# shz9/viprs

Hardware: AMD Instinct MI355X
Metric: SNP-updates/sec/E-step (1M SNPs, ~1700 LD blocks) (higher is better)
Workload: dtype f32

## Files before the change

### viprs_amd/csrc/estep_panel.h

```cpp
#pragma once
#include <type_traits>

#include "device_math.h"
#include "kernels_common.h"
#include "panel_loads.h"
#include "panel_models.h"

#ifndef PANEL_MIN_WAVES
#define PANEL_MIN_WAVES 2
#endif

namespace viprs {

#ifdef VIPRS_SWEEP_TRACE
__device__ unsigned long long g_sweep_trace[1 << 15][4];
__device__ unsigned int g_sweep_trace_n;
#endif

#ifdef VIPRS_PANEL_PROFILE
#define PPROF(slot, cond) do { if (TEAM && item == 0 && member < 2 && lane == 0 && p < 64 && (cond)) s_pprof[p][slot] = (unsigned)wall_clock64(); } while (0)
#else
#define PPROF(slot, cond) do { } while (0)
#endif

template <typename U> __host__ __device__ constexpr int panel_cols() { return sizeof(U) == 4 ? 4 : 8; }
template <typename U> __host__ __device__ constexpr int panel_team_cols() {
#ifdef PANEL_TEAM_CPL_F32
    return sizeof(U) == 4 ? PANEL_TEAM_CPL_F32 : 4;
#else
    return sizeof(U) == 4 ? 2 : 4;
#endif
}

constexpr int kFormSym = 1, kFormMirror = 2;

template <typename U, typename MODEL, int FORM, int NW, bool TEAM, int CPL>
__device__ __forceinline__ void panel_role(const EStepArgs<float>& A0, const int qcap, float* __restrict__ smem, const int wg) {
    constexpr bool MIR = FORM == kFormMirror;
    constexpr bool SUMS = FORM != kFormSym;
    const PanelLds lds(qcap, MODEL::kLaneParallel && !is_wide_mixture<MODEL>::value, MIR);
    float* lq = smem + lds.q();
    float* la = smem + lds.a();
    float* lT = smem + lds.diag_tiles();
    float* lTo = smem + lds.offdiag_tile();
    float* lmx = smem + lds.mix();
    float* led = smem + lds.ed();
    float* ls = smem + lds.s();
#ifdef PANEL_TEAM_STRIP_DEPTH
    constexpr int kDepth = TEAM ? PANEL_TEAM_STRIP_DEPTH : kStripRowsInFlight;
#else
    constexpr int kDepth = TEAM ? (kPanel / RawRow<U, CPL>::kWords < kPanel ? kPanel / RawRow<U, CPL>::kWords : kPanel) : kStripRowsInFlight;
#endif
    __shared__ int s_blk;
    __shared__ int s_tdone;
    __shared__ int s_ddone;

    const int tid = threadIdx.x;
    const int wave = __builtin_amdgcn_readfirstlane(tid >> 6);
    const int lane = tid & 63;
    const U* __restrict__ ldd = static_cast<const U*>(A0.ld_dense);
    ExpTab tab;
    tab.init();
    unsigned long long my_skipped = 0;
    const float dq = A0.dq;
    const int n_models = max(1, A0.n_active);

    constexpr int kSW = kPanel * CPL;
    const int TS = TEAM ? A0.team_size : 1;
    const int team = TEAM ? wg / TS : 0;
    const int member = TEAM ? wg % TS : 0;
    int team_iter = 0;

    for (;;) {
        int item;
        if (TEAM) {
            item = team + team_iter * A0.n_teams;
            ++team_iter;
        } else {
            if (tid == 0) {
                int it = atomicAdd(A0.counter, 1);
                if (A0.bottom_mod > 0 && it < A0.n_blocks * n_models) {
                    const bool bottom = (wg % A0.bottom_mod) == A0.bottom_mod - 1;
                    it = bottom ? A0.n_blocks * n_models - 1 - atomicAdd(A0.counter + 2, 1) : atomicAdd(A0.counter + 1, 1);
                }
                s_blk = it;
            }
            __syncthreads();
            item = s_blk;
            __syncthreads();
        }
        if (item >= A0.n_blocks * n_models) break;
        const int blk = item / n_models, model_slot = item - blk * n_models;
        if constexpr (IsGridColumn<MODEL>::value) {
            if (A0.group_cols) {
                const int on = A0.group_cols[(int64_t)A0.blk_group[blk] * A0.width + A0.active[model_slot]];
                if (__builtin_amdgcn_readfirstlane(on) == 0) continue;
            }
        }
        const EStepArgs<float> A = select_model(A0, model_slot);

        const BlockDesc bd = A.blocks[blk];
        const int64_t s0 = bd.start;
        const int b = bd.size;
#ifdef VIPRS_SWEEP_TRACE
        const unsigned long long trace_t0 = wall_clock64();
#endif
        unsigned long long* __restrict__ gran =
            TEAM ? A.granules + ((int64_t)model_slot * A.granule_rows + bd.gr_off) * kPanel : nullptr;
        const int stride = bd.stride;
        const U* __restrict__ base = ldd + bd.ld_off;
        const int np = (b + kPanel - 1) / kPanel;
        const int bpad = np * kPanel;
        const int nstrips_all = (bpad + kSW - 1) / kSW;
        const int n_own = TEAM ? (nstrips_all - member + TS - 1) / TS : nstrips_all;
        auto own = [&](int c) { return !TEAM || ((c / kSW) % TS) == member; };
        auto loc = [&](int c) { return TEAM ? ((c / kSW) / TS) * kSW + (c % kSW) : c; };
        auto glob = [&](int li) { return TEAM ? ((li / kSW) * TS + member) * kSW + (li % kSW) : li; };

        for (int li = tid; li < (TEAM ? n_own * kSW : bpad) + kStrip; li += NW * 64) {
            const int c = glob(li);
            const bool in = (!TEAM || li < n_own * kSW) && c < b;
            lq[li] = in ? A.q[s0 + c] : 0.0f;
            if (SUMS) ls[li] = 0.0f;
        }
        if (tid == 0) { s_tdone = 0; s_ddone = 0; }
        for (int i = tid; i < kPanel * kPanel / 4; i += NW * 64) {
            const int row = i >> 4, tcol = (i & 15) * 4;
            *reinterpret_cast<float4*>(lT + row * kPanel + tcol) = load4<U>(base + (int64_t)min(row, b - 1) * stride + tcol);
        }
        __syncthreads();

        float a_prev = 0.0f;

        typename MODEL::In nxt_in{};
        if (wave == 0) {
            const bool live0 = lane < b;
            nxt_in = MODEL::load(A, s0 + (live0 ? lane : 0), live0);
        }

#ifdef VIPRS_PANEL_PROFILE
        __shared__ unsigned s_pprof[64][8];
#endif
        if (wave == 0) {
#ifdef PANEL_CHAIN_PRIO
        __builtin_amdgcn_s_setprio(PANEL_CHAIN_PRIO);
#endif
        for (int p = 0; p < np + 1; ++p) {
            PPROF(0, true);
            {
                if (p < np) {
                    const int r0 = p * kPanel;
                    const int nrows = min(kPanel, b - r0);
                    const int64_t j = s0 + r0 + lane;
                    const bool live = lane < nrows;
                    const typename MODEL::In in = nxt_in;
                    {
                        const int rn = r0 + kPanel + lane;
                        const bool ln = rn < b;
                        nxt_in = MODEL::load(A, s0 + (ln ? rn : 0), ln);
                    }

                    float qc;
                    float q_own = 0.0f;
                    if (own(r0)) qc = lq[loc(r0 + lane)];
                    else qc = (r0 + lane < b) ? A.q[s0 + r0 + lane] : 0.0f;
                    if (TEAM && p >= 2 && (((p * kPanel) / kSW) % TS) != member) {
                        unsigned long long g = 0;
#ifdef PANEL_TIMING_NO_HANDOFF_WAIT
                        if (false)
#endif
                        for (unsigned spins = 0;; ++spins) {
                            g = __hip_atomic_load(gran + (int64_t)p * kPanel + lane, __ATOMIC_RELAXED,
                                                  __HIP_MEMORY_SCOPE_AGENT);
                            if (__all((unsigned)(g >> 32) == A.tag_base + (unsigned)(p + 1))) break;
                            if (spins > (1u << 22)) {
                                if (lane == 0) atomicExch(A.error, 1);
                                break;
                            }
                            if ((spins & 1023u) == 1023u &&
                                __hip_atomic_load(A.error, __ATOMIC_RELAXED, __HIP_MEMORY_SCOPE_AGENT) != 0) break;
                            __builtin_amdgcn_s_sleep(8);
                        }
                        qc = __uint_as_float((unsigned)g);
                    }
                    PPROF(1, true);
                    if (p > 0) {
                        {
                            float trow[kPanel];
#pragma unroll
                            for (int k = 0; k < kPanel; ++k) trow[k] = lTo[k * kPanel + lane];
                            if constexpr (sizeof(U) < 4 || MODEL::kLaneParallel) {
                                const float4* __restrict__ av4 = reinterpret_cast<const float4*>(la + ((p - 1) & 1) * kPanel);
                                float4 av[kPanel / 4];
#pragma unroll
                                for (int i = 0; i < kPanel / 4; ++i) av[i] = av4[i];
#pragma unroll
                                for (int k = 0; k < kPanel; ++k) {
                                    const float4 t = av[k >> 2];
                                    const float ak = (k & 3) == 0 ? t.x : (k & 3) == 1 ? t.y : (k & 3) == 2 ? t.z : t.w;
                                    qc = __builtin_fmaf(trow[k], ak, qc);
                                }
                            } else {
#pragma unroll
                                for (int k = 0; k < kPanel; ++k) qc = __builtin_fmaf(trow[k], rl(a_prev, k), qc);
                            }
                        }
                    }

                    {
                        if (lane == 0) *reinterpret_cast<volatile int*>(&s_tdone) = p + 1;
                    }
                    PPROF(2, true);
                    if constexpr (is_wide_mixture<MODEL>::value) {
                        constexpr int KMAX = MODEL::kMax;
                        const int K = in.K;
                        const int kc = min(lane, K - 1);
                        const bool comp = lane < K;
                        float dvec = 0.0f, avec = 0.0f;
                        const int64_t jlast = s0 + b - 1;
                        auto cptr = [&](const float* __restrict__ arr, int jj) {
                            return arr + min(s0 + r0 + jj, jlast) * K + kc;
                        };
                        static_assert(kChainPrefetch == 16 && kPanel == 64, "window indexing");
                        float rmm[kChainPrefetch], rsv[kChainPrefetch], rul[kChainPrefetch];
                        float rvec = in.beta - qc;
                        const float* __restrict__ DtW = lT + (p & 1) * kPanel * kPanel + lane;
#pragma unroll
                        for (int k = 0; k < kChainPrefetch; ++k) {
                            rmm[k] = *cptr(A.mu_mult, k);
                            rsv[k] = *cptr(A.shvt, k);
                            rul[k] = *cptr(A.u_logs, k);
                        }
#pragma unroll 1
                        for (int g = 0; g < kPanel / kChainPrefetch; ++g) {
#pragma unroll
                        for (int k = 0; k < kChainPrefetch; ++k) {
                            const int jj = kChainPrefetch * g + k;
                            const float drow_jj = DtW[jj * kPanel];
                            const float cmm = rmm[k], csv = rsv[k], cul = rul[k];
                            {
                                rmm[k] = *cptr(A.mu_mult, jj + kChainPrefetch);
                                rsv[k] = *cptr(A.shvt, jj + kChainPrefetch);
                                rul[k] = *cptr(A.u_logs, jj + kChainPrefetch);
                            }
                            const float lnp = rl(in.lnp, jj), eta_old = rl(in.eta_old, jj);
                            const float r = rl(rvec, jj);
                            const float mu = cmm * r;
                            const float t = csv * mu;
                            float u = __builtin_fmaf(t, t, cul);
                            u = (lane == K) ? lnp : u;
                            float mx = dpp_max_shr<1>(u);
                            mx = dpp_max_shr<2>(mx);
                            mx = dpp_max_shr<4>(mx);
                            mx = dpp_max_shr<8>(mx);
                            const float m_lo = rl(mx, 15), m_hi = rl(mx, K);
                            mx = (K >= 16) ? fmaxf(m_lo, m_hi) : m_hi;
                            float e = expf_glibc_nonpos<kLookupPerLane>(u - mx, tab);
                            e = (lane <= K) ? e : 0.0f;
                            static_assert((KMAX + 1) % 8 == 0, "chunks of 8 terms");
                            float ssum = 0.0f;
#pragma unroll
                            for (int c = 0; c < (KMAX + 1) / 8; ++c) {
                                int et[8];
#pragma unroll
                                for (int i = 0; i < 8; ++i) et[i] = __builtin_amdgcn_readlane(__float_as_int(e), 8 * c + i);
                                pin_sgprs(et);
#pragma unroll
                                for (int i = 0; i < 8; ++i) ssum = (c == 0 && i == 0) ? __int_as_float(et[0]) : ssum + __int_as_float(et[i]);
                            }
                            const float gam = comp ? e / ssum : 0.0f;
                            float d = -eta_old;
#pragma unroll
                            for (int c = 0; c < (KMAX + 1) / 8; ++c) {
                                int gt[8];
                                float mb[8];
#pragma unroll
                                for (int i = 0; i < 8; ++i) {
                                    gt[i] = __builtin_amdgcn_readlane(__float_as_int(gam), 8 * c + i);
                                    mb[i] = rl(mu, 8 * c + i);
                                }
                                pin_sgprs(gt);
#pragma unroll
                                for (int i = 0; i < 8; ++i) d = __builtin_fmaf(__int_as_float(gt[i]), mb[i], d);
                            }
                            const bool livej = jj < nrows;
                            const float a = livej ? dq * d : 0.0f;
                            if (comp && livej && member == 0) {
                                const int64_t o = (s0 + r0 + jj) * K + lane;
                                A.var_mu[o] = mu;
                                A.var_gamma[o] = gam;
                            }
                            int l = lane;
                            asm volatile("" : "+v"(l));
                            const bool me = (l == jj);
                            dvec = me ? d : dvec;
                            avec = me ? a : avec;
                            if (MIR) q_own = me ? qc : q_own;
                            qc = __builtin_fmaf(drow_jj, a, qc);
                            rvec = in.beta - qc;
                            if (!MIR) qc = (me && livej) ? qc - d : qc;
                        }
                        }
                        if (member == 0 && live) {
                            A.eta_diff[j] = dvec;
                            if (TEAM) stage_store(A.eta_out + j, in.eta_old + dvec); else A.eta[j] = in.eta_old + dvec;
                        }
                        a_prev = avec;
                        if (SUMS) led[(p & 1) * kPanel + lane] = live ? dvec : 0.0f;
                    } else if constexpr (MODEL::kLaneParallel) {
                        const int K = in.K;
                        float* __restrict__ Lmm = lmx;
                        float* __restrict__ Lsv = lmx + kPanel * kPanelMaxK;
                        float* __restrict__ Lul = lmx + 2 * kPanel * kPanelMaxK;
                        float* __restrict__ Lmu = lmx + 3 * kPanel * kPanelMaxK;
                        float* __restrict__ Lga = lmx + 4 * kPanel * kPanelMaxK;
#pragma unroll
                        for (int k = 0; k < kPanelMaxK; ++k) {
                            if (k < K) {
                                Lmm[lane * K + k] = in.mm[k];
                                Lsv[lane * K + k] = in.sv[k];
                                Lul[lane * K + k] = in.ulog[k];
                            }
                        }
                        __builtin_amdgcn_wave_barrier();
                        const int kc = min(lane, K - 1);
                        float cmm = Lmm[kc], csv = Lsv[kc], cul = Lul[kc];
                        float dvec = 0.0f, avec = 0.0f;
                        auto run_panel = [&](auto rounds_c, auto k4_c) {
                        constexpr int ROUNDS = decltype(rounds_c)::value;
                        constexpr bool K4 = decltype(k4_c)::value;
                        float rvec = in.beta - qc;
                        static_assert(kChainPrefetch == 16 && kPanel == 64, "group indexing");
                        const float* __restrict__ Dt = lT + (p & 1) * kPanel * kPanel + lane;
#pragma unroll 1
                        for (int g = 0; g < kPanel / kChainPrefetch; ++g) {
#pragma unroll
                        for (int k = 0; k < kChainPrefetch; ++k) {
                            const int jj = kChainPrefetch * g + k;
                            const float drow_jj = Dt[jj * kPanel];
                            const int jn = (jj + 1 < kPanel) ? jj + 1 : jj;
                            const float nmm = Lmm[jn * K + kc], nsv = Lsv[jn * K + kc], nul = Lul[jn * K + kc];
                            const float lnp = rl(in.lnp, jj), eta_old = rl(in.eta_old, jj);
                            const float r = rl(rvec, jj);
                            const float mu = cmm * r;
                            const float t = csv * mu;
                            float u = __builtin_fmaf(t, t, cul);
                            u = (lane == K) ? lnp : u;
                            float mub[ROUNDS];
#pragma unroll
                            for (int i = 0; i < ROUNDS; ++i) mub[i] = rl(mu, i);
                            float mx;
                            if constexpr (K4) {
                                int ut[5];
#pragma unroll
                                for (int i = 0; i < 5; ++i) ut[i] = __builtin_amdgcn_readlane(__float_as_int(u), i);
                                pin_sgprs(ut);
                                mx = __int_as_float(ut[0]);
#pragma unroll
                                for (int i = 1; i <= 4; ++i) mx = fmaxf(mx, __int_as_float(ut[i]));
                            } else {
                                mx = dpp_max_shr<1>(u);
                                mx = dpp_max_shr<2>(mx);
                                mx = dpp_max_shr<4>(mx);
                                mx = dpp_max_shr<8>(mx);
                                mx = rl(mx, K);
                            }
                            const float e = softmax_exp<MODEL::kExact, kLookupPerLane>(u - mx, tab);
                            const float e_t = (K4 || lane <= K) ? e : 0.0f;
                            int et[ROUNDS + 1];
#pragma unroll
                            for (int i = 0; i <= ROUNDS; ++i) et[i] = __builtin_amdgcn_readlane(__float_as_int(e_t), i);
                            pin_sgprs(et);
                            float ssum = __int_as_float(et[0]);
#pragma unroll
                            for (int i = 1; i <= ROUNDS; ++i) ssum += __int_as_float(et[i]);
                            const float gam = softmax_div<MODEL::kExact>(e, ssum);
                            const float gam_t = (K4 || lane < K) ? gam : 0.0f;
                            int gt[ROUNDS];
#pragma unroll
                            for (int i = 0; i < ROUNDS; ++i) gt[i] = __builtin_amdgcn_readlane(__float_as_int(gam_t), i);
                            pin_sgprs(gt);
                            float d = -eta_old;
#pragma unroll
                            for (int i = 0; i < ROUNDS; ++i) d = __builtin_fmaf(__int_as_float(gt[i]), mub[i], d);
                            const bool livej = jj < nrows;
                            const float a = livej ? dq * d : 0.0f;
                            if (lane < K) {
                                Lmu[jj * K + lane] = mu;
                                Lga[jj * K + lane] = gam;
                            }
                            int l = lane;
                            asm volatile("" : "+v"(l));
                            const bool me = (l == jj);
                            dvec = me ? d : dvec;
                            avec = me ? a : avec;
                            if (MIR) q_own = me ? qc : q_own;
                            qc = __builtin_fmaf(drow_jj, a, qc);
                            rvec = in.beta - qc;
                            if (!MIR) qc = (me && livej) ? qc - d : qc;
                            cmm = nmm; csv = nsv; cul = nul;
                        }
                        }
                        };
                        if (K == 4) run_panel(std::integral_constant<int, 4>{}, std::true_type{});
                        else if (K < 4) run_panel(std::integral_constant<int, 4>{}, std::false_type{});
                        else run_panel(std::integral_constant<int, kPanelMaxK>{}, std::false_type{});
                        __builtin_amdgcn_wave_barrier();
                        if (member == 0) {
                            const int64_t o = (s0 + r0) * K;
                            for (int i = lane; i < nrows * K; i += 64) {
                                A.var_mu[o + i] = Lmu[i];
                                A.var_gamma[o + i] = Lga[i];
                            }
                            if (live) {
                                A.eta_diff[j] = dvec;
                                if (TEAM) stage_store(A.eta_out + j, in.eta_old + dvec); else A.eta[j] = in.eta_old + dvec;
                            }
                        }
                        a_prev = avec;
                        if (SUMS) led[(p & 1) * kPanel + lane] = live ? dvec : 0.0f;
                    } else {
                        float qcap_v = 0.0f;
                        const float* __restrict__ Dt = lT + (p & 1) * kPanel * kPanel + lane;
                        unsigned long long lane_bit = 1ull;
                        float qf = qc;
    #pragma unroll
                        for (int jj = 0; jj < kPanel; ++jj) {
                            const float dr = Dt[jj * kPanel];
                            const float d = MODEL::template delta<kLookupLane>(in, qf, tab, jj);
                            const float dz = (MODEL::kHasSkip && fabsf(d) < Eps<float>::value) ? 0.0f : d;
                            const float az = dq * dz;
                            const float sa = rl(az, jj);
                            const float sdz = rl(dz, jj);
                            qcap_v = sel_mask(qcap_v, qc, lane_bit);
                            qf = __builtin_fmaf(dr, sa, qc);
                            qc = !MIR ? sel_mask(qf, qf - sdz, lane_bit) : qf;
                            asm volatile("s_lshl_b64 %0, %0, 1" : "+s"(lane_bit) : : "scc");
                        }
                        q_own = qcap_v;

                        PPROF(3, true);
                        bool skipped_lane;
                        float d_lane = 0.0f;
                        a_prev = MODEL::template finish<TEAM>(A, j, in, qcap_v, tab, live, member == 0, skipped_lane, &d_lane);
                        my_skipped += __popcll(__ballot(skipped_lane));
                        if (SUMS) led[(p & 1) * kPanel + lane] = d_lane;
                    }
                    la[(p & 1) * kPanel + lane] = a_prev;
                    if (own(r0)) lq[loc(r0 + lane)] = MIR ? q_own : qc;
                    PPROF(4, true);
                }
            }
            __syncthreads();
        }
        } else {
        for (int p = 0; p < np + 1; ++p) {
            {
                const int uw = wave - 1;
                auto stage_tiles = [&]() {
                if (p + 1 < np) {
                    float* __restrict__ T = lT + ((p + 1) & 1) * kPanel * kPanel;
                    const int trow = lane >> 4, tcol = (lane & 15) * 4;
                    const int row_base = (p + 1) * kPanel;
                    constexpr int kGroups = (kPanel / 4 + NW - 2) / (NW - 1);
                    float4 v[kGroups];
#pragma unroll
                    for (int g = 0; g < kGroups; ++g) {
                        const int row = 4 * min(uw + g * (NW - 1), kPanel / 4 - 1) + trow;
                        v[g] = load4<U>(base + (int64_t)min(row_base + row, b - 1) * stride + (p + 1) * kPanel + tcol);
                    }
                    float4 w[kGroups];
                    {
#pragma unroll
                        for (int g = 0; g < kGroups; ++g) {
                            const int row = 4 * min(uw + g * (NW - 1), kPanel / 4 - 1) + trow;
                            w[g] = load4<U>(base + (int64_t)min(p * kPanel + row, b - 1) * stride + (p + 1) * kPanel + tcol);
                        }
                    }
                    if (MIR && p > 0) {
                        while (*reinterpret_cast<volatile int*>(&s_ddone) < p) __builtin_amdgcn_s_sleep(1);
                    }
#pragma unroll
                    for (int g = 0; g < kGroups; ++g) {
                        const int i = uw + g * (NW - 1);
                        if (i < kPanel / 4) *reinterpret_cast<float4*>(T + (4 * i + trow) * kPanel + tcol) = v[g];
                    }
                    {
                        while (*reinterpret_cast<volatile int*>(&s_tdone) < p + 1) __builtin_amdgcn_s_sleep(1);
#pragma unroll
                        for (int g = 0; g < kGroups; ++g) {
                            const int i = uw + g * (NW - 1);
                            if (i < kPanel / 4) *reinterpret_cast<float4*>(lTo + (4 * i + trow) * kPanel + tcol) = w[g];
                        }
                    }
                }
                };
                const int pp = p - 1;
                const int rr0 = pp * kPanel;
                const int last_row = min(kPanel, b - rr0) - 1;
                const float avec = p > 0 ? la[(pp & 1) * kPanel + lane] : 0.0f;
                const int nstrips = (bpad + kSW - 1) / kSW;
                const bool any_a = __ballot(avec != 0.0f) != 0;
                const float edvec = (MIR && p > 0) ? led[(pp & 1) * kPanel + lane] : 0.0f;
                const bool any_ed = MIR && __ballot(edvec != 0.0f) != 0;
                const int s_pri = ((p + 1) * kPanel) / kSW;
                const int n_mine = (nstrips - member + TS - 1) / TS;
                auto do_strip = [&](int k) {
                    int st = member + k * TS, kl = k;
                    if (TEAM) {
                        const int k_pri = (s_pri % TS == member) ? (s_pri - member) / TS : 0;
                        kl = (k + k_pri) % n_mine;
                        st = member + kl * TS;
                    }
                    const int c = st * kSW + CPL * lane;
                    float* __restrict__ lq_c = lq + (TEAM ? kl * kSW + CPL * lane : c);
                    const int cp = c >> 6;
#if defined(PANEL_TIMING_NO_SECOND_PASS) && PANEL_TIMING_NO_SECOND_PASS + 0 >= 2
                    const bool active = (c < b) && cp > p;
#else
                    const bool active = (c < b) && cp != pp && cp != p;
#endif
                    auto hand_off = [&]() {
                        if (TEAM && st == s_pri && p + 1 < np && p + 1 >= 2) {
                            __builtin_amdgcn_wave_barrier();
                            const float v = lq[loc((p + 1) * kPanel + lane)];
                            const unsigned long long g =
                                ((unsigned long long)(A.tag_base + (unsigned)(p + 2)) << 32) | (unsigned long long)__float_as_uint(v);
                            __hip_atomic_store(gran + (int64_t)(p + 1) * kPanel + lane, g, __ATOMIC_RELAXED,
                                               __HIP_MEMORY_SCOPE_AGENT);
                        }
                    };
                    if constexpr (MIR) {
                        const bool left = cp < pp;
                        float* __restrict__ tgt = left ? ls + (TEAM ? kl * kSW + CPL * lane : c) : lq_c;
                        const bool any_l = __ballot(active && left) != 0, any_r = __ballot(active && !left) != 0;
                        if (any_l && any_r) {
                            const float fvec = left ? 1.0f : dq;
                            if (any_ed && active) {
                                if (last_row == kPanel - 1)
                                    strip_update<U, CPL, true, kDepth, true>(base + (int64_t)rr0 * stride + c, stride, last_row, edvec, tgt, fvec);
                                else
                                    strip_update<U, CPL, false, kDepth, true>(base + (int64_t)rr0 * stride + c, stride, last_row, edvec, tgt, fvec);
                            }
                        } else {
                            float mvec = any_l ? edvec : avec;
                            asm volatile("" : "+v"(mvec));
                            if ((any_l ? any_ed : any_a) && active) {
                                if (last_row == kPanel - 1)
                                    strip_update<U, CPL, true, kDepth>(base + (int64_t)rr0 * stride + c, stride, last_row, mvec, tgt);
                                else
                                    strip_update<U, CPL, false, kDepth>(base + (int64_t)rr0 * stride + c, stride, last_row, mvec, tgt);
                            }
                        }
                        if (k == uw) PPROF(6, wave == 1);
                        hand_off();
                    } else {
                        if (any_a && active) {
                            if (last_row == kPanel - 1)
                                strip_update<U, CPL, true, kDepth>(base + (int64_t)rr0 * stride + c, stride, last_row, avec, lq_c);
                            else
                                strip_update<U, CPL, false, kDepth>(base + (int64_t)rr0 * stride + c, stride, last_row, avec, lq_c);
                        }
                        if (k == uw) PPROF(6, wave == 1);
                        hand_off();
                    }
                };
                if (MIR && p > 0 && uw == NW - 2) {
#ifdef PANEL_TIMING_NO_SECOND_PASS
                    if (false) {
#else
                    if (any_ed && own(rr0)) {
#endif
                        float* __restrict__ sp = ls + loc(rr0 + lane);
                        *sp = diag_lower_update(lT + (pp & 1) * kPanel * kPanel, edvec, *sp, lane);
                    }
                    if (lane == 0) *reinterpret_cast<volatile int*>(&s_ddone) = p;
                }
                stage_tiles();
                PPROF(5, wave == 1);
                if (p > 0) {
                    for (int k = uw; k < n_mine; k += NW - 1) do_strip(k);
                }
            }
            PPROF(7, wave == 1);
            __syncthreads();
        }
        }
#ifdef VIPRS_PANEL_PROFILE
        if (TEAM && item == 0 && member < 2 && tid == 0) {
            for (int p = 0; p < np && p < 64; p += (p < 4 || p > np - 4) ? 1 : 8) {
                const unsigned t = s_pprof[p][0];
                printf("m%d phase %2d @%7u: granule %4d T-apply %4d loop %5d replay %5d end %5d | upd: staged %5d pri %5d all %5d (x10ns)\n",
                       member, p, t - s_pprof[0][0], (int)(s_pprof[p][1] - t), (int)(s_pprof[p][2] - t), (int)(s_pprof[p][3] - t),
                       (int)(s_pprof[p][4] - t), (int)(s_pprof[p][4] - t), (int)(s_pprof[p][5] - t), (int)(s_pprof[p][6] - t),
                       (int)(s_pprof[p][7] - t));
            }
        }
#endif
        {
            for (int li = tid; li < (TEAM ? n_own * kSW : b); li += NW * 64) {
                const int i = glob(li);
                if (i < b) {
                    const float v = SUMS ? lq[li] + A.dq * ls[li] : lq[li];
                    if (TEAM) stage_store(A.q_out + s0 + i, v); else A.q[s0 + i] = v;
                }
            }
        }
        if (TEAM) {
            asm volatile("s_waitcnt vmcnt(0)" ::: "memory");
            __syncthreads();
            if (tid == 0) s_blk = (atomicAdd(A.arrive + item, 1) == TS - 1) ? 1 : 0;
            __syncthreads();
            const bool last = s_blk != 0;
            if (last) {
                for (int i = tid; i < b; i += NW * 64) {
                    A.eta[s0 + i] = __hip_atomic_load(A.eta_out + s0 + i, __ATOMIC_RELAXED, __HIP_MEMORY_SCOPE_AGENT);
                    A.q[s0 + i] = __hip_atomic_load(A.q_out + s0 + i, __ATOMIC_RELAXED, __HIP_MEMORY_SCOPE_AGENT);
                }
                if (tid == 0) atomicExch(A.arrive + item, 0);
            }
        }
        __syncthreads();
#ifdef VIPRS_SWEEP_TRACE
        if (tid == 0) {
            const unsigned k = atomicAdd(&g_sweep_trace_n, 1u);
            if (k < (1u << 15)) {
                g_sweep_trace[k][0] = ((unsigned long long)blockIdx.x << 32) | (unsigned)(TEAM ? 1 : 0);
                g_sweep_trace[k][1] = (unsigned long long)b;
                g_sweep_trace[k][2] = trace_t0;
                g_sweep_trace[k][3] = wall_clock64();
            }
        }
#endif
    }
    if (lane == 0 && my_skipped && member == 0) atomicAdd(A0.skipped, my_skipped);
}

struct SweepArgs {
    EStepArgs<float> cls[3];
    int32_t qcap[3];
    int32_t n_wg[2];
    int32_t narrow0;
    int32_t* done;
    unsigned long long* skipped_last;
};

template <typename U, typename MODEL, int FORM, int NW, int CPL>
__global__ __launch_bounds__(NW * 64, PANEL_MIN_WAVES) void estep_sweep_kernel(SweepArgs S) {
    extern __shared__ __attribute__((aligned(16))) float smem[];
    const int wg = blockIdx.x;
    const int team_cls = wg < S.n_wg[0] ? 0 : (wg < S.n_wg[0] + S.n_wg[1] ? 1 : 2);
    if (team_cls < 2) {
        constexpr bool kNarrowForm = FORM == kFormMirror && sizeof(U) < 4;
        constexpr int CPL_N = (MODEL::kLaneParallel || !kNarrowForm) ? CPL : panel_team_cols<U>();
        const int wg_t = wg - (team_cls ? S.n_wg[0] : 0);
        if (CPL_N != CPL && team_cls == 0 && S.narrow0)
            panel_role<U, MODEL, FORM, NW, true, CPL_N>(S.cls[0], S.qcap[0], smem, wg_t);
        else
            panel_role<U, MODEL, FORM, NW, true, CPL>(S.cls[team_cls], S.qcap[team_cls], smem, wg_t);
        __syncthreads();
    }
    if (S.cls[2].n_blocks > 0) panel_role<U, MODEL, FORM, NW, false, CPL>(S.cls[2], S.qcap[2], smem, wg);
    __syncthreads();
    if (threadIdx.x == 0) {
        if (atomicAdd(S.done, 1) == (int)gridDim.x - 1) {
            S.cls[2].counter[0] = 0; S.cls[2].counter[1] = 0; S.cls[2].counter[2] = 0;
            atomicExch(S.skipped_last, atomicExch(S.cls[2].skipped, 0ull));
            atomicExch(S.done, 0);
        }
    }
}

}
```

### viprs_amd/csrc/panel_loads.h

```cpp
#pragma once
#include "kernels_common.h"

namespace viprs {

template <typename U> __device__ __forceinline__ float4 load4(const U* p);
template <> __device__ __forceinline__ float4 load4<float>(const float* p) {
    return *reinterpret_cast<const float4*>(p);
}
template <> __device__ __forceinline__ float4 load4<int8_t>(const int8_t* p) {
    const int w = *reinterpret_cast<const int*>(p);
    return make_float4((float)(int8_t)(w), (float)(int8_t)(w >> 8), (float)(int8_t)(w >> 16),
                       (float)(int8_t)(w >> 24));
}
template <> __device__ __forceinline__ float4 load4<int16_t>(const int16_t* p) {
    const int2 w = *reinterpret_cast<const int2*>(p);
    return make_float4((float)(int16_t)(w.x), (float)(int16_t)(w.x >> 16), (float)(int16_t)(w.y),
                       (float)(int16_t)(w.y >> 16));
}

template <int N> __device__ __forceinline__ void pin_sgprs(int (&v)[N]) {
    static_assert(N == 4 || N == 5 || N == 8 || N == 9, "chain lengths of the K <= 8 mixture step");
    if constexpr (N == 4) asm volatile("" : "+s"(v[0]), "+s"(v[1]), "+s"(v[2]), "+s"(v[3]));
    if constexpr (N == 5) asm volatile("" : "+s"(v[0]), "+s"(v[1]), "+s"(v[2]), "+s"(v[3]), "+s"(v[4]));
    if constexpr (N == 8) asm volatile("" : "+s"(v[0]), "+s"(v[1]), "+s"(v[2]), "+s"(v[3]), "+s"(v[4]), "+s"(v[5]), "+s"(v[6]), "+s"(v[7]));
    if constexpr (N == 9) asm volatile("" : "+s"(v[0]), "+s"(v[1]), "+s"(v[2]), "+s"(v[3]), "+s"(v[4]), "+s"(v[5]), "+s"(v[6]), "+s"(v[7]),
                                       "+s"(v[8]));
}
template <int N> __device__ __forceinline__ float dpp_max_shr(float x) {
    float r;
    if (N == 1) asm("s_nop 1\n\tv_max_f32_dpp %0, %1, %1 row_shr:1 row_mask:0xf bank_mask:0xf" : "=v"(r) : "v"(x), "0"(x));
    if (N == 2) asm("s_nop 1\n\tv_max_f32_dpp %0, %1, %1 row_shr:2 row_mask:0xf bank_mask:0xf" : "=v"(r) : "v"(x), "0"(x));
    if (N == 4) asm("s_nop 1\n\tv_max_f32_dpp %0, %1, %1 row_shr:4 row_mask:0xf bank_mask:0xf" : "=v"(r) : "v"(x), "0"(x));
    if (N == 8) asm("s_nop 1\n\tv_max_f32_dpp %0, %1, %1 row_shr:8 row_mask:0xf bank_mask:0xf" : "=v"(r) : "v"(x), "0"(x));
    return r;
}

__device__ __forceinline__ float sel_mask(float a, float b, unsigned long long m) {
    float r;
    asm("v_cndmask_b32_e64 %0, %1, %2, %3" : "=v"(r) : "v"(a), "v"(b), "s"(m));
    return r;
}

__device__ __forceinline__ void stage_store(float* p, float v) {
    __hip_atomic_store(p, v, __ATOMIC_RELAXED, __HIP_MEMORY_SCOPE_AGENT);
}

__device__ __forceinline__ float rl(float v, int lane) {
    return __int_as_float(__builtin_amdgcn_readlane(__float_as_int(v), lane));
}

template <typename U, int CPL> struct RawRow {
    static constexpr int kWords = CPL * (int)sizeof(U) / 4;
    static_assert(CPL * sizeof(U) % 4 == 0 && (kWords == 1 || kWords == 2 || kWords == 4), "1, 2 or 4 dwords per lane and row");
    unsigned w[kWords];
    __device__ __forceinline__ float get(int i) const {
        if constexpr (sizeof(U) == 4) return __uint_as_float(w[i]);
        else if constexpr (sizeof(U) == 1) return static_cast<float>(static_cast<int8_t>(w[i >> 2] >> (8 * (i & 3))));
        else return static_cast<float>(static_cast<int16_t>(w[i >> 1] >> (16 * (i & 1))));
    }
};
template <typename U, int CPL> __device__ __forceinline__ RawRow<U, CPL> load_raw(const U* p) {
    RawRow<U, CPL> r;
    if constexpr (RawRow<U, CPL>::kWords == 1) {
        r.w[0] = *reinterpret_cast<const unsigned*>(p);
    } else if constexpr (RawRow<U, CPL>::kWords == 2) {
        const uint2 t = *reinterpret_cast<const uint2*>(p);
        r.w[0] = t.x; r.w[1] = t.y;
    } else {
        const uint4 t = *reinterpret_cast<const uint4*>(p);
        r.w[0] = t.x; r.w[1] = t.y; r.w[2] = t.z; r.w[3] = t.w;
    }
    return r;
}

constexpr int kChainPrefetch = 16;
#ifndef PANEL_STRIP_DEPTH
#define PANEL_STRIP_DEPTH 16
#endif
constexpr int kStripRowsInFlight = PANEL_STRIP_DEPTH;


template <typename U, int CPL, bool FULL, int DEPTH = kStripRowsInFlight, bool MIXED = false>
__device__ __forceinline__ void strip_update(const U* __restrict__ rowp, int stride, int last_row, float avec,
                                             float* __restrict__ lq_c, float fvec = 1.0f) {
    static_assert(kPanel % DEPTH == 0, "panel must be a whole number of prefetch groups");
    float qv[CPL];
#pragma unroll
    for (int i = 0; i < CPL; ++i) qv[i] = lq_c[i];
    RawRow<U, CPL> buf[DEPTH];
#pragma unroll
    for (int k = 0; k < DEPTH; ++k)
        buf[k] = load_raw<U, CPL>(rowp + (int64_t)(FULL ? k : min(k, last_row)) * stride);
#pragma unroll 1
    for (int g = 0; g < kPanel / DEPTH - 1; ++g) {
#pragma unroll
        for (int k = 0; k < DEPTH; ++k) {
            const RawRow<U, CPL> v = buf[k];
            const int rn = DEPTH * (g + 1) + k;
            buf[k] = load_raw<U, CPL>(rowp + (int64_t)(FULL ? rn : min(rn, last_row)) * stride);
            const float a = MIXED ? fvec * rl(avec, DEPTH * g + k) : rl(avec, DEPTH * g + k);
#pragma unroll
            for (int i = 0; i < CPL; ++i) qv[i] = __builtin_fmaf(v.get(i), a, qv[i]);
            __builtin_amdgcn_sched_barrier(0);
        }
    }
#pragma unroll
    for (int k = 0; k < DEPTH; ++k) {
        const RawRow<U, CPL> v = buf[k];
        const float a = MIXED ? fvec * rl(avec, kPanel - DEPTH + k) : rl(avec, kPanel - DEPTH + k);
#pragma unroll
        for (int i = 0; i < CPL; ++i) qv[i] = __builtin_fmaf(v.get(i), a, qv[i]);
    }
#pragma unroll
    for (int i = 0; i < CPL; ++i) lq_c[i] = qv[i];
}

__device__ __forceinline__ float diag_lower_update(const float* __restrict__ tile, float edvec, float sv, int lane) {
#pragma unroll 16
    for (int jr = 0; jr < kPanel; ++jr) {
        const float t = __builtin_fmaf(tile[jr * kPanel + lane], rl(edvec, jr), sv);
        sv = lane < jr ? t : sv;
    }
    return sv;
}

}
```

Measured before the change: 1.565 billion.

## Compact nonzero panel rows into a list and skip zero-multiplier LD rows

Before each strip update, a ballot over the panel's multiplier vector builds a compacted list of rows whose coefficient is nonzero, using mbcnt and ds_permute. When that count fits under a threshold, a new strip_update_rows variant streams only those rows of the LD matrix, rounded up to whole prefetch groups, instead of all 64. This cuts memory traffic when few SNPs changed in a panel, which is common in sparse mixture models. The cost is extra permute and readlane work per panel, plus gathered row loads that are less regular.

```diff
diff --git a/viprs_amd/csrc/estep_panel.h b/viprs_amd/csrc/estep_panel.h
--- a/viprs_amd/csrc/estep_panel.h
+++ b/viprs_amd/csrc/estep_panel.h
@@ -503,6 +503,13 @@
                 const bool any_a = __ballot(avec != 0.0f) != 0;
                 const float edvec = (MIR && p > 0) ? led[(pp & 1) * kPanel + lane] : 0.0f;
                 const bool any_ed = MIR && __ballot(edvec != 0.0f) != 0;
+                constexpr bool kRowLists = !MODEL::kLaneParallel && !is_wide_mixture<MODEL>::value;
+                constexpr int kRowsMax = kRowLists ? kPanel - kDepth : 0;
+                RowList rows_a{0, 0, 0.0f}, rows_ed{0, 0, 0.0f};
+                if constexpr (kRowLists) {
+                    rows_a = build_row_list(avec, last_row, lane, kRowsMax);
+                    if (MIR) rows_ed = build_row_list(edvec, last_row, lane, kRowsMax);
+                }
                 const int s_pri = ((p + 1) * kPanel) / kSW;
                 const int n_mine = (nstrips - member + TS - 1) / TS;
                 auto do_strip = [&](int k) {
@@ -537,16 +544,24 @@
                         if (any_l && any_r) {
                             const float fvec = left ? 1.0f : dq;
                             if (any_ed && active) {
-                                if (last_row == kPanel - 1)
+                                if (kRowsMax > 0 && rows_ed.n <= kRowsMax)
+                                    strip_update_rows<U, CPL, kDepth, true>(base + (int64_t)rr0 * stride + c, stride, rows_ed.n, rows_ed.idx, rows_ed.mul, tgt, fvec);
+                                else if (last_row == kPanel - 1)
                                     strip_update<U, CPL, true, kDepth, true>(base + (int64_t)rr0 * stride + c, stride, last_row, edvec, tgt, fvec);
                                 else
                                     strip_update<U, CPL, false, kDepth, true>(base + (int64_t)rr0 * stride + c, stride, last_row, edvec, tgt, fvec);
                             }
                         } else {
                             float mvec = any_l ? edvec : avec;
+                            int ivec = any_l ? rows_ed.idx : rows_a.idx;
+                            float lvec = any_l ? rows_ed.mul : rows_a.mul;
+                            const int n_rows = any_l ? rows_ed.n : rows_a.n;
                             asm volatile("" : "+v"(mvec));
+                            if constexpr (kRowLists) asm volatile("" : "+v"(ivec), "+v"(lvec));
                             if ((any_l ? any_ed : any_a) && active) {
-                                if (last_row == kPanel - 1)
+                                if (kRowsMax > 0 && n_rows <= kRowsMax)
+                                    strip_update_rows<U, CPL, kDepth>(base + (int64_t)rr0 * stride + c, stride, n_rows, ivec, lvec, tgt);
+                                else if (last_row == kPanel - 1)
                                     strip_update<U, CPL, true, kDepth>(base + (int64_t)rr0 * stride + c, stride, last_row, mvec, tgt);
                                 else
                                     strip_update<U, CPL, false, kDepth>(base + (int64_t)rr0 * stride + c, stride, last_row, mvec, tgt);
@@ -556,7 +571,9 @@
                         hand_off();
                     } else {
                         if (any_a && active) {
-                            if (last_row == kPanel - 1)
+                            if (kRowsMax > 0 && rows_a.n <= kRowsMax)
+                                strip_update_rows<U, CPL, kDepth>(base + (int64_t)rr0 * stride + c, stride, rows_a.n, rows_a.idx, rows_a.mul, lq_c);
+                            else if (last_row == kPanel - 1)
                                 strip_update<U, CPL, true, kDepth>(base + (int64_t)rr0 * stride + c, stride, last_row, avec, lq_c);
                             else
                                 strip_update<U, CPL, false, kDepth>(base + (int64_t)rr0 * stride + c, stride, last_row, avec, lq_c);
diff --git a/viprs_amd/csrc/panel_loads.h b/viprs_amd/csrc/panel_loads.h
--- a/viprs_amd/csrc/panel_loads.h
+++ b/viprs_amd/csrc/panel_loads.h
@@ -115,6 +115,66 @@
     for (int i = 0; i < CPL; ++i) lq_c[i] = qv[i];
 }
 
+struct RowList {
+    int n;
+    int idx;
+    float mul;
+};
+__device__ __forceinline__ RowList build_row_list(float mvec, int last_row, int lane, int max_n) {
+    RowList L;
+    const unsigned long long mask = __ballot(mvec != 0.0f);
+    L.n = __popcll(mask);
+    L.idx = 0;
+    L.mul = 0.0f;
+    if (L.n > 0 && L.n <= max_n) {
+        const int rank = __builtin_amdgcn_mbcnt_hi((unsigned)(mask >> 32), __builtin_amdgcn_mbcnt_lo((unsigned)mask, 0));
+        const int dest = ((mask >> lane) & 1ull) ? rank : L.n + (lane - rank);
+        const int idx = __builtin_amdgcn_ds_permute(dest << 2, lane);
+        const float mul = __int_as_float(__builtin_amdgcn_ds_bpermute(idx << 2, __float_as_int(mvec)));
+        const int idx_last = __builtin_amdgcn_readlane(idx, L.n - 1);
+        L.idx = min(lane < L.n ? idx : idx_last, last_row);
+        L.mul = lane < L.n ? mul : 0.0f;
+    }
+    asm volatile("" : "+v"(L.idx), "+v"(L.mul));
+    return L;
+}
+
+template <typename U, int CPL, int DEPTH = kStripRowsInFlight, bool MIXED = false>
+__device__ __forceinline__ void strip_update_rows(const U* __restrict__ rowp, int stride, int n, int idxvec, float mulvec,
+                                                  float* __restrict__ lq_c, float fvec = 1.0f) {
+    static_assert(kPanel % DEPTH == 0, "panel must be a whole number of prefetch groups");
+    float qv[CPL];
+#pragma unroll
+    for (int i = 0; i < CPL; ++i) qv[i] = lq_c[i];
+    const int ng = (n + DEPTH - 1) / DEPTH;
+    RawRow<U, CPL> buf[DEPTH];
+#pragma unroll
+    for (int k = 0; k < DEPTH; ++k)
+        buf[k] = load_raw<U, CPL>(rowp + (int64_t)__builtin_amdgcn_readlane(idxvec, k) * stride);
+#pragma unroll 1
+    for (int g = 0; g < ng - 1; ++g) {
+#pragma unroll
+        for (int k = 0; k < DEPTH; ++k) {
+            const RawRow<U, CPL> v = buf[k];
+            buf[k] = load_raw<U, CPL>(rowp + (int64_t)__builtin_amdgcn_readlane(idxvec, DEPTH * (g + 1) + k) * stride);
+            const float a = MIXED ? fvec * rl(mulvec, DEPTH * g + k) : rl(mulvec, DEPTH * g + k);
+#pragma unroll
+            for (int i = 0; i < CPL; ++i) qv[i] = __builtin_fmaf(v.get(i), a, qv[i]);
+            __builtin_amdgcn_sched_barrier(0);
+        }
+    }
+    const int g_last = DEPTH * (ng - 1);
+#pragma unroll
+    for (int k = 0; k < DEPTH; ++k) {
+        const RawRow<U, CPL> v = buf[k];
+        const float a = MIXED ? fvec * rl(mulvec, g_last + k) : rl(mulvec, g_last + k);
+#pragma unroll
+        for (int i = 0; i < CPL; ++i) qv[i] = __builtin_fmaf(v.get(i), a, qv[i]);
+    }
+#pragma unroll
+    for (int i = 0; i < CPL; ++i) lq_c[i] = qv[i];
+}
+
 __device__ __forceinline__ float diag_lower_update(const float* __restrict__ tile, float edvec, float sv, int lane) {
 #pragma unroll 16
     for (int jr = 0; jr < kPanel; ++jr) {
```

After: 1.553 billion. Within noise of the previous version (-0.7%).
